# burlachenkok/flpytorch

Hardware: AMD Instinct MI355X
Metric: gradient-codec encode+reduce GB/s (device-resident), [N,D] fp32; % HBM peak (higher is better)
Workload: dtype f32; 1 GPU; C3 topk:1% N=1024/GPU D=10000000; codec=topk:1%, clients_per_gpu=1024, clients_total=1024, D=10000000, K=100000, rows_alloc=contiguous, parallelism=client-shard dp1

## Files before the change

### flpytorch_amd/csrc/select.hip

```cpp
#include <stdlib.h>

#include <atomic>
#include <map>
#include <mutex>
#include <vector>

#include "chunks.hpp"
#include "randk_tree.hpp"

namespace flc {

constexpr uint32_t ALL = 0xFFFFFFFFu;
constexpr uint32_t F_OVERFLOW = 1u, F_SHORT = 2u, F_TIES = 4u, F_EXACT = 8u;
constexpr uint32_t F_RESIDENT = 16u;
constexpr uint32_t F_REPAIR = 32u;
constexpr int SMAX = 16384;
constexpr int HBINS = 2048;
constexpr uint32_t TIECAP = HBINS;
constexpr int CS_SH = 64;
constexpr int64_t CS_FEW = 16;
constexpr int CS_ST = 8;
constexpr int CS_LCAP = 2048;
constexpr int RS_U = 16;
#ifndef FLC_RS_NG
// ... 3 lines not shown
constexpr int RS_NG_MAX = 16;
static_assert(RS_NG >= 1 && RS_NG <= RS_NG_MAX, "FLC_RS_NG: 1..16 groups");
constexpr int RS_GLOB = 0, RS_GEN = 32, RS_GAVE = 64, RS_CCNT = 96, RS_CDONE = 112, RS_GRP = 128;
constexpr int RS_XGRP = RS_GRP + 32 * RS_NG_MAX;
constexpr int RS_ABV = RS_XGRP + 32 * RS_NG_MAX;
constexpr int RS_CAP = 2048;
constexpr int RS_SS = 8192;
#ifndef FLC_RS_SR
#define FLC_RS_SR 1
#endif
constexpr int RS_SR = FLC_RS_SR;
#ifndef FLC_RS_STPOL
#define FLC_RS_STPOL 2
#endif
#ifndef FLC_RS_GACQ
#define FLC_RS_GACQ 1
#endif
#ifndef FLC_RS_POLLAB
#define FLC_RS_POLLAB 1
#endif
#ifndef FLC_RS_DONE
#define FLC_RS_DONE 1
#endif
#ifndef FLC_RS_RANKFIRST
#define FLC_RS_RANKFIRST 0
#endif
#ifndef FLC_RS_PROBE_NOCOUNT
#define FLC_RS_PROBE_NOCOUNT 0
#endif
#ifndef FLC_RS_G0REL
#define FLC_RS_G0REL 1
#endif
#ifndef FLC_RS_FENCE
#define FLC_RS_FENCE 0
#endif
#ifndef FLC_RS_SPEC
#define FLC_RS_SPEC 1
#endif
constexpr int RS_HREP = RS_ABV + 32 * RS_NG_MAX;
constexpr int RS_HSPEC = RS_HREP + 3 * RS_NG * HBINS;
constexpr int RS_CLIST = RS_HSPEC + 3 * RS_NG * HBINS;
constexpr int RS_TCNT = RS_CLIST + 2 * RS_CAP;
constexpr int RS_GMAX = 1024;
constexpr int RS_CS = 4;
constexpr int RS_CNUM = RS_TCNT + 2 * RS_GMAX;
constexpr int RS_CREG = RS_CNUM + RS_GMAX;
#ifdef FLC_RS_PRINT
constexpr int RS_PROBE = RS_CREG + 2 * RS_CS * RS_GMAX;
constexpr int RS_CTL = RS_PROBE + 4096;
#else
constexpr int RS_CTL = RS_CREG + 2 * RS_CS * RS_GMAX;
#endif
#ifndef FLC_RS_SPECST
#define FLC_RS_SPECST 0
#endif
#ifndef FLC_CS_LIST
#define FLC_CS_LIST 1
#endif
#ifndef FLC_CS_TWO_MAXD
#define FLC_CS_TWO_MAXD (int64_t(64) << 20)
#endif

struct SelWs {
    uint2* tab;
    uint32_t* ent_idx;
    float* ent_val;
    uint32_t* rowcnt;
    uint32_t* flags;
    uint32_t* thr;
    uint32_t* prefix;
    uint32_t* krem;
    uint32_t* tieprefix;
    uint32_t* tiecut;
    uint32_t* hist;
    uint32_t* worklist;
    uint32_t* nwork;
    uint32_t* cursor;
    uint32_t* cstate;
    uint64_t* clist;
    uint32_t* carrive;
    uint32_t* shcnt;
    uint32_t* zm;
    float* part;
    int64_t cap;
    uint32_t tie_hi;
};

__device__ __host__ inline uint32_t tie_pref(uint32_t ix, uint32_t hi) { return hi ? ix : ~ix; }
__device__ __host__ inline uint32_t tie_all(uint32_t hi) { return hi ? 0u : 0xFFFFFFFFu; }


__device__ inline void lds_bar() {
    asm volatile("s_waitcnt lgkmcnt(0)" ::: "memory");
    __builtin_amdgcn_s_barrier();
    asm volatile("" ::: "memory");
}
template <bool RAW>
__device__ inline void blk_bar() {
    if (RAW) lds_bar();
    else __syncthreads();
}
template <bool RAW = false>
__device__ inline void hist_find_at(const uint32_t* h, uint32_t k, uint32_t& bin, uint32_t& above,
                                    uint32_t* scratch , int t, bool own) {
    uint32_t local[8];
    uint32_t s = 0;
#pragma unroll
    for (int q = 0; q < 8; ++q) { local[q] = own ? h[HBINS - 1 - (t * 8 + q)] : 0u; s += local[q]; }
    if (t == 0) { scratch[256] = 0; scratch[257] = 0; }
    const int lane = t & 63, w = t >> 6;
    uint32_t inc = s;
#pragma unroll
    for (int off = 1; off < 64; off <<= 1) {
        const uint32_t v = __shfl_up(inc, off, 64);
        inc += lane >= off ? v : 0u;
    }
    if (own && lane == 63) scratch[w] = inc;
    blk_bar<RAW>();
    uint32_t before = 0;
    if (own)
        for (int q = 0; q < w; ++q) before += scratch[q];
    uint32_t incl = own ? before + inc : 0u, excl = incl - s;
    if (own && excl < k && incl >= k) {
        uint32_t run = excl;
#pragma unroll
        for (int q = 0; q < 8; ++q) {
            if (run + local[q] >= k) {
                scratch[256] = (uint32_t)(HBINS - 1 - (t * 8 + q));
                scratch[257] = run;
                break;
            }
            run += local[q];
        }
    }
    blk_bar<RAW>();
    bin = scratch[256];
    above = scratch[257];
    blk_bar<RAW>();
}
template <int NB>
__device__ inline void hist_find_n(const uint32_t* h, uint32_t k, uint32_t& bin, uint32_t& above, bool& found,
                                   uint32_t* scratch ) {
    constexpr int PER = NB / 256;
    static_assert(NB % 256 == 0, "256 threads scan NB / 256 bins each");
    const int t = (int)threadIdx.x;
    const bool own = t < 256;
    uint32_t local[PER];
    uint32_t s = 0;
#pragma unroll
    for (int q = 0; q < PER; ++q) { local[q] = own ? h[NB - 1 - (t * PER + q)] : 0u; s += local[q]; }
    if (t == 0) { scratch[256] = 0; scratch[257] = 0; scratch[258] = 0; }
    const int lane = t & 63, w = t >> 6;
    uint32_t inc = s;
#pragma unroll
    for (int off = 1; off < 64; off <<= 1) {
        const uint32_t v = __shfl_up(inc, off, 64);
        inc += lane >= off ? v : 0u;
    }
    if (own && lane == 63) scratch[w] = inc;
    __syncthreads();
    uint32_t before = 0;
    if (own)
        for (int q = 0; q < w; ++q) before += scratch[q];
    const uint32_t incl = own ? before + inc : 0u, excl = incl - s;
    if (own && excl < k && incl >= k) {
        uint32_t run = excl;
// ... 715 lines not shown
            __amdgpu_buffer_rsrc_t rsn;
            if (sub + 1 < FGS) {
                rsn = chunk_rsrc(rows.row_s(row), j0 + CHUNK, d);
            } else if (nit < items) {
                item_at(nit, nrow, nc);
                rsn = chunk_rsrc(rows.row_s(nrow), nc * CHUNK, d);
            } else {
                rsn = __builtin_amdgcn_make_buffer_rsrc(const_cast<float*>(rows.row_s(row)), (short)0, 0, 0x00020000);
            }
            const uint32_t cnt0 = cnt;
            __amdgpu_buffer_rsrc_t ro;
            if constexpr (LONE != 0) ro = chunk_rsrc(zout, j0, d);
            uint32_t lb = (uint32_t)j0 + (uint32_t)lane * 4u;
            asm volatile("" : "+v"(lb));
#pragma unroll
            for (int L = 0; L < 16; ++L) {
                const int P = L + RING - 1;
                ring[P % RING] = P < 16 ? load_q(rs, lane, P) : load_q(rsn, lane, P - 16);
                const float4 x = ring[L % RING];
                if constexpr (LONE != 0) {
                    typedef unsigned int u4v __attribute__((ext_vector_type(4)));
                    const u4v z = {0u, 0u, 0u, 0u};
                    __builtin_amdgcn_raw_buffer_store_b128(z, ro, lane * 16, L * 1024, 0);
                }
                const uint32_t jl = lb + (uint32_t)(L * 256);
                const float vq[4] = {x.x, x.y, x.z, x.w};
#pragma unroll
                for (int q = 0; q < 4; ++q) {
                    if (FLC_TK_PROBE == 3) { cnt += __float_as_uint(vq[q]) == 0x7F800001u ? 1u : 0u; continue; }
                    const bool f = mag_key(vq[q]) >= T;
                    const uint64_t m = __ballot(f);
                    if (FLC_TK_PROBE != 1 && f) {
                        const uint32_t pre = __builtin_amdgcn_mbcnt_hi((uint32_t)(m >> 32), __builtin_amdgcn_mbcnt_lo((uint32_t)m, 0u));
                        uint32_t sb = sla + min(cnt, (uint32_t)GCAP) * 4u;
                        asm volatile("" : "+s"(sb));
                        asm volatile("ds_write2st64_b32 %0, %1, %2 offset1:%3" ::"v"(sb + pre * 4u),
                                     "v"(jl + q), "v"(__float_as_uint(vq[q])), "i"(SROW * 4 / 256) : "memory");
                    }
                    cnt += (uint32_t)__popcll(m);
                }
            }
            ccp |= (uint64_t)min(cnt - cnt0, 0xFFFFu) << (16 * (c - cg0));
            rs = rsn;
        }
        if (pv) finish(par ^ 1);
        uint32_t res = 0;
        const int64_t shard = shards > 1 ? (cg0 / FGS) % shards : 0;
        if (cnt && cnt <= GCAP && lane == 0)
            res = atomicAdd(shards > 1 ? &ws.shcnt[(row * shards + shard) * RCS] : &ws.rowcnt[(row) * RCS], cnt);
        pv = true; prow = row; pc0 = cg0; pcc = ccp; ptot = cnt; pres = res; pseg = shard;
        __builtin_amdgcn_fence(__ATOMIC_SEQ_CST, "wavefront");
        par ^= 1;
        it = nit;
        row = nrow;
        c = nc;
    }
    __builtin_amdgcn_fence(__ATOMIC_SEQ_CST, "wavefront");
    finish(par ^ 1);
}

#ifndef FLC_TK_WG
#define FLC_TK_WG 1
#endif
#ifndef FLC_TK_WG_NL
#define FLC_TK_WG_NL 4
#endif
#ifndef FLC_TK_WG_RING
#define FLC_TK_WG_RING FLC_TK_RING
#endif
#ifndef FLC_TK_WG_STPOL
#define FLC_TK_WG_STPOL 17
#endif
#ifndef FLC_TK_WG_WPE
#define FLC_TK_WG_WPE 4
#endif
__device__ inline uint32_t lds_addr(const void* p) {
    return (uint32_t)(size_t)(const __attribute__((address_space(3))) void*)p;
}
__device__ inline uint32_t lds_peek(uint32_t addr) {
    uint32_t v;
    asm volatile("ds_read_b32 %0, %1\n\ts_waitcnt lgkmcnt(0)" : "=&v"(v) : "v"(addr) : "memory");
    return __builtin_amdgcn_readfirstlane(v);
}
template <int RING, int NL>
__global__ __launch_bounds__((NL + 1) * 64) __attribute__((amdgpu_waves_per_eu(FLC_TK_WG_WPE))) void k_topk_filter_fast_wg(RowSrc rows, int64_t n, int64_t r0, int64_t rn, int64_t rb, int64_t d,
                                                                        SelWs ws) {
    static_assert(16 % RING == 0, "ring must divide the 16 loads of a chunk");
    constexpr int FGS = 4;
    constexpr int SROW = GCAP + 64;
    __shared__ __attribute__((aligned(16))) uint32_t st[2][NL][2 * SROW];
    __shared__ __attribute__((aligned(16))) uint32_t hs[2][NL][4];
    __shared__ uint32_t fr[2];
    const int lane = threadIdx.x & 63;
    const int wv = __builtin_amdgcn_readfirstlane(threadIdx.x >> 6);
    if (threadIdx.x < 2 * NL * 4) (&hs[0][0][0])[threadIdx.x] = 0;
    if (threadIdx.x < 2) fr[threadIdx.x] = 0;
    __syncthreads();
    const int64_t C = nchunks(d);
    const int64_t G = (C + FGS * NL - 1) / (FGS * NL);
    const int64_t items = rn * G;
    const int64_t stride = gridDim.x;
    int64_t it = blockIdx.x;
    if (it >= items) return;
    auto item_at = [&](int64_t t, int64_t& r, int64_t& cc) {
        const int64_t blk = t / (rb * G), rem = t - blk * rb * G;
        const int64_t bn = min(rb, rn - blk * rb);
        const int64_t g = rem / bn;
        r = r0 + blk * rb + (rem - g * bn);
        cc = g * (FGS * NL);
    };
    if (wv == NL) {
        for (uint32_t k = 0; it < items; it += stride, ++k) {
            const int b = k & 1;
            int64_t row, c0;
            item_at(it, row, c0);
            const uint32_t fa = lds_addr(&hs[b][min(lane, NL - 1)][3]);
            for (;;) {
                uint32_t f;
                asm volatile("ds_read_b32 %0, %1\n\ts_waitcnt lgkmcnt(0)" : "=&v"(f) : "v"(fa) : "memory");
                if (__ballot(f != k + 1) == 0) break;
                __builtin_amdgcn_s_sleep(4);
            }
            uint32_t pre[NL], tot[NL], sum = 0;
            uint64_t cc[NL];
            bool allfit = true;
#pragma unroll
            for (int w = 0; w < NL; ++w) {
                const uint4 h = *reinterpret_cast<const uint4*>(hs[b][w]);
                cc[w] = (uint64_t)h.x | ((uint64_t)h.y << 32);
                tot[w] = h.z;
                pre[w] = sum;
                sum += tot[w] <= GCAP ? tot[w] : 0u;
                allfit = allfit && tot[w] <= GCAP;
            }
            uint32_t base = 0;
            bool fits = true;
            if (sum) {
                uint32_t res = 0;
                if (lane == 0) res = atomicAdd(&ws.rowcnt[row * RCS], sum);
                base = __shfl(res, 0, WAVE);
                fits = (int64_t)base + sum <= ws.cap;
            }
            if (lane < FGS * NL && c0 + lane < C) {
                uint32_t off = 0, cu = 0;
                bool gf = false;
#pragma unroll
                for (int w = 0; w < NL; ++w)
                    if ((lane >> 2) == w) {
                        off = pre[w];
                        gf = tot[w] <= GCAP;
#pragma unroll
                        for (int u = 0; u < FGS; ++u) {
                            const uint32_t x = (uint32_t)(cc[w] >> (16 * u)) & 0xFFFFu;
                            off += u < (lane & 3) ? x : 0u;
                            cu = u == (lane & 3) ? x : cu;
                        }
                    }
                ws.tab[(c0 + lane) * n + row] = make_uint2(base + off, fits && gf ? cu : 0u);
            }
            if (!(fits && allfit) && lane == 0) atomicOr(&ws.flags[row], F_OVERFLOW);
#pragma unroll
            for (int w = 0; w < NL; ++w)
                tk_copy_out<FLC_TK_WG_STPOL>(st[b][w], st[b][w] + SROW, ws, n, row, base + pre[w], tot[w], fits && tot[w] <= GCAP, lane,
                            (int64_t)blockIdx.x * NL + w);
            asm volatile("s_waitcnt lgkmcnt(0)\n\tds_write_b32 %0, %1" ::"v"(lds_addr(&fr[b])), "v"(k + 1) : "memory");
        }
        return;
    }
    float4 ring[RING];
    int64_t row, c;
    item_at(it, row, c);
    c += wv * FGS;
    auto rs = chunk_rsrc(rows.row_s(row), c * CHUNK, d);
#pragma unroll
    for (int L = 0; L < RING - 1; ++L) {
        ring[L] = load_q(rs, lane, L);
        __builtin_amdgcn_sched_barrier(0);
    }
    for (uint32_t k = 0; it < items; ++k) {
        const int b = k & 1;
        if (k >= 2) {
            const uint32_t fa = lds_addr(&fr[b]);
            while (lds_peek(fa) != k - 1) __builtin_amdgcn_s_sleep(2);
        }
        const uint32_t T = max(sload(ws.thr + row), 1u);
        const int64_t nit = it + stride;
        const uint32_t sla = __builtin_amdgcn_readfirstlane(lds_addr(st[b][wv]));
        uint32_t cnt = 0;
        uint64_t ccp = 0;
        const int64_t cg0 = c;
        int64_t nrow = row, nc = c;
#pragma unroll
        for (int sub = 0; sub < FGS; ++sub, ++c) {
            const int64_t j0 = c * CHUNK;
            __amdgpu_buffer_rsrc_t rsn;
            if (sub + 1 < FGS) {
                rsn = chunk_rsrc(rows.row_s(row), j0 + CHUNK, d);
            } else if (nit < items) {
                item_at(nit, nrow, nc);
                nc += wv * FGS;
                rsn = chunk_rsrc(rows.row_s(nrow), nc * CHUNK, d);
            } else {
                rsn = __builtin_amdgcn_make_buffer_rsrc(const_cast<float*>(rows.row_s(row)), (short)0, 0, 0x00020000);
            }
            const uint32_t cnt0 = cnt;
            uint32_t lb = (uint32_t)j0 + (uint32_t)lane * 4u;
            asm volatile("" : "+v"(lb));
#pragma unroll
            for (int L = 0; L < 16; ++L) {
                const int P = L + RING - 1;
                ring[P % RING] = P < 16 ? load_q(rs, lane, P) : load_q(rsn, lane, P - 16);
                const float4 x = ring[L % RING];
                const uint32_t jl = lb + (uint32_t)(L * 256);
                const float vq[4] = {x.x, x.y, x.z, x.w};
#pragma unroll
                for (int q = 0; q < 4; ++q) {
                    const bool f = mag_key(vq[q]) >= T;
                    const uint64_t m = __ballot(f);
                    if (f) {
                        const uint32_t pre = __builtin_amdgcn_mbcnt_hi((uint32_t)(m >> 32), __builtin_amdgcn_mbcnt_lo((uint32_t)m, 0u));
                        uint32_t sb = sla + min(cnt, (uint32_t)GCAP) * 4u;
                        asm volatile("" : "+s"(sb));
                        asm volatile("ds_write2st64_b32 %0, %1, %2 offset1:%3" ::"v"(sb + pre * 4u),
                                     "v"(jl + q), "v"(__float_as_uint(vq[q])), "i"(SROW * 4 / 256) : "memory");
                    }
                    cnt += (uint32_t)__popcll(m);
                }
            }
            ccp |= (uint64_t)min(cnt - cnt0, 0xFFFFu) << (16 * (c - cg0));
            rs = rsn;
        }
        if (lane == 0)
            asm volatile("ds_write_b64 %0, %1\n\tds_write_b32 %0, %2 offset:8\n\tds_write_b32 %0, %3 offset:12"
                         ::"v"(lds_addr(hs[b][wv])), "v"(ccp), "v"(cnt), "v"(k + 1) : "memory");
        it = nit;
        row = nrow;
        c = nc;
    }
}

template <bool FULLROW>
__global__ __launch_bounds__(256) void k_radix_hist(RowSrc rows, int64_t n, int64_t d, int p, SelWs ws) {
    __shared__ uint32_t h[HBINS];
    constexpr int64_t BLK = 65536;
    const int64_t nrows = FULLROW ? (int64_t)(*ws.nwork) : n;
    const int64_t maxlen = FULLROW ? d : ws.cap;
    const int64_t bpr = (maxlen + BLK - 1) / BLK;
    const int64_t items = nrows * bpr;
// ... 1884 lines not shown
            }
            const u4v ov = {o[0], o[1], o[2], o[3]};
            __builtin_amdgcn_raw_buffer_store_b128(ov, ro, voff, u * RS_NT * 16, FLC_RS_STPOL);
        }
    }
    RS_STAMP(11);
    (void)bar;
    }
    goto done;
leave:
    if (t == 0) {
        __builtin_amdgcn_fence(__ATOMIC_RELEASE, "agent");
    }
    if (!rep_s) count_out();
    __syncthreads();
    if (rep_s) {
        const RsExit ex = ex_s;
        if (t == 0) {
            const uint64_t t0 = (uint64_t)wall_clock64();
            for (;;) {
                uint32_t out_n = 0;
                for (int r = 0; r < RS_NG; ++r)
                    out_n += __hip_atomic_load(ex.ctl + RS_XGRP + 32 * r, __ATOMIC_RELAXED, __HIP_MEMORY_SCOPE_AGENT);
                if (out_n - ex.xbase >= ex.G - 1u || (uint64_t)wall_clock64() - t0 >= 64 * ex.spin) break;
                __builtin_amdgcn_s_sleep(8);
            }
            __builtin_amdgcn_fence(__ATOMIC_ACQUIRE, "agent");
        }
        __syncthreads();
        rs_repair(ex.x, ex.d, ex.K, ex.tie_hi, ex.thr, ex.krem, ex.tiecut, ex.flags, ex.out, ex.ctl, h, scratch, wsum);
        __syncthreads();
        if (t == 0) __builtin_amdgcn_fence(__ATOMIC_RELEASE, "agent");
        count_out();
    }
done:;
#ifdef FLC_RS_PRINT
    asm volatile("s_waitcnt vmcnt(0)" ::: "memory");
    __syncthreads();
    RS_STAMP(12);
    if (t == 0 && G <= 256u) {
        uint64_t* pr = reinterpret_cast<uint64_t*>(ex_s.ctl + RS_PROBE);
        const int ks[8] = {FLC_RS_TLK, 13};
        for (int k = 0; k < 8; ++k) __hip_atomic_store(pr + k * 256 + g, stamp[ks[k]], __ATOMIC_RELAXED, __HIP_MEMORY_SCOPE_AGENT);
    }
#endif
}

static int64_t host_chunks(int64_t d) { return (d + CHUNK - 1) / CHUNK; }

int64_t sel_capacity(int codec, int64_t d, int64_t K) {
    if (codec == FLC_RANDK) return std::max<int64_t>(K, 1);
    int64_t cap = 2 * K + 2 * CHUNK;
    cap = std::min<int64_t>(std::max<int64_t>(cap, 1), std::max<int64_t>(d, 1));
    return (cap + 3) & ~int64_t(3);
}

static SelWs carve_sel(void* base, int codec, int64_t n, int64_t d, int64_t K, size_t* bytes) {
    Carver cv(base);
    const int64_t C = std::max<int64_t>(host_chunks(d), 1), nn = std::max<int64_t>(n, 1);
    SelWs s;
    s.tie_hi = 0;
    s.cap = sel_capacity(codec, d, K);
    s.tab = cv.take<uint2>((size_t)C * nn);
    s.ent_idx = cv.take<uint32_t>((size_t)nn * s.cap);
    s.ent_val = cv.take<float>((size_t)nn * s.cap);
    s.rowcnt = cv.take<uint32_t>((size_t)nn * RCS);
    s.flags = cv.take<uint32_t>(nn);
    s.thr = cv.take<uint32_t>(nn);
    s.prefix = cv.take<uint32_t>(nn);
    s.krem = cv.take<uint32_t>(nn);
    s.worklist = cv.take<uint32_t>(nn);
    s.nwork = cv.take<uint32_t>(4);
    s.zm = cv.take<uint32_t>((size_t)C * (CHUNK / 32));
    s.part = codec == FLC_TOPK ? cv.take<float>((size_t)C * CHUNK) : nullptr;
    if (codec == FLC_TOPK) {
        s.tieprefix = cv.take<uint32_t>((size_t)C * nn);
        s.tiecut = cv.take<uint32_t>(nn);
        s.hist = cv.take<uint32_t>((size_t)nn * HBINS);
        s.cursor = nullptr;
        s.cstate = cv.take<uint32_t>((size_t)nn * CS_ST);
        s.clist = cv.take<uint64_t>((size_t)std::min<int64_t>(nn, CS_FEW) * CS_LCAP);
        s.carrive = cv.take<uint32_t>((size_t)nn * RCS);
        s.shcnt = cv.take<uint32_t>((size_t)std::min<int64_t>(nn, CS_FEW) * CS_SH * RCS);
    } else {
        s.tieprefix = nullptr;
        s.tiecut = nullptr;
        s.hist = nullptr;
        s.cursor = cv.take<uint32_t>((size_t)std::max<int64_t>(C, RK_SB) * nn);
        s.cstate = nullptr;
        s.clist = nullptr;
        s.carrive = nullptr;
        s.shcnt = nullptr;
    }
    if (bytes) *bytes = cv.bytes();
    return s;
}

size_t randk_device_workspace(int64_t n, int64_t d);

size_t sel_workspace(const flc_codec_params* prm, int64_t n, int64_t d) {
    size_t b = 0;
    carve_sel(nullptr, prm->codec, n, d, prm->k, &b);
    if (prm->codec == FLC_RANDK) b += randk_device_workspace(n, d);
    return b;
}

static int grid_stride_blocks(int64_t items, int64_t cap = 4096) {
    return (int)std::max<int64_t>(1, std::min<int64_t>(items, cap));
}

static int accum_parts() {
    static const int p = [] {
        const char* e = tuning_env("FLC_ACCUM_PARTS");
        const int v = e ? atoi(e) : 0;
        return (v == 1 || v == 2 || v == 4) ? v : 0;
    }();
    return p;
}

static bool assign_fold() {
    static const bool v = [] { const char* e = tuning_env("FLC_ASSIGN_FOLD"); return e && atoi(e) == 1; }();
    return v;
}

static bool cs_single() {
    static const bool v = [] { const char* e = tuning_env("FLC_CS_SINGLE"); return e && atoi(e) == 1; }();
    return v;
}

#ifndef FLC_LONE_PATH
#define FLC_LONE_PATH 2
#endif
#ifndef FLC_RS_EVREC
#define FLC_RS_EVREC 1
#endif
#ifndef FLC_RS_COOP
#define FLC_RS_COOP 0
#endif
struct RsCtx {
    uint32_t* ctl = nullptr;
    uint32_t seq = 0;
    uint32_t xcum = 0;
    hipStream_t last = nullptr;
    hipEvent_t done = nullptr;
};
static std::mutex g_rs_mu;
static std::map<int, RsCtx> g_rs_ctx;
static std::atomic<int> g_rs_dbg_mult{1};
static std::atomic<long long> g_rs_dbg_spin{0};
int rs_debug(int mult, int64_t spin_ticks) {
    if (mult < 1 || mult > 64 || spin_ticks < 0) { set_error("flc_debug_resident: mult 1..64, spin >= 0"); return FLC_ERR_ARG; }
    g_rs_dbg_mult.store(mult);
    g_rs_dbg_spin.store((long long)spin_ticks);
    return FLC_OK;
}
static int rs_cus() {
    static int cu[64] = {0};
    int dev = 0;
    if (hipGetDevice(&dev) != hipSuccess || dev < 0 || dev >= 64) return 0;
    if (!cu[dev]) {
        int c = 0;
        if (hipDeviceGetAttribute(&c, hipDeviceAttributeMultiprocessorCount, dev) != hipSuccess) return 0;
        cu[dev] = c;
    }
    return cu[dev];
}
static int lone_path() {
    static const int v = [] { const char* e = tuning_env("FLC_LONE_PATH"); return e ? atoi(e) : FLC_LONE_PATH; }();
    return v;
}

static int filter_group() {
    static const int g = [] {
        const char* e = tuning_env("FLC_FILTER_GS");
        return (e && atoi(e) == 2) ? 2 : 4;
    }();
    return g;
}

template <int FGS>
static void launch_filter(RowSrc rows, int64_t n, int64_t r0, int64_t rn, int64_t d, SelWs ws, hipStream_t st,
                          int shards, float* zout = nullptr) {
    const int64_t waves = rn * ((nchunks(d) + FGS - 1) / FGS);
    const int gw = (int)std::max<int64_t>(1, std::min<int64_t>((waves + 3) / 4, 32768));
    static const int64_t rb = [] {
        const char* e = tuning_env("FLC_TK_RB");
        return e ? std::max<int64_t>(1, atoll(e)) : (int64_t)64;
    }();
    ProfScope _pv(FGS == 4 ? "k_topk_filter_g4" : "k_topk_filter_g2", st);
    if constexpr (FGS == 4 && FLC_TK_WG != 0 && FLC_TK_PROBE != 1 && FLC_TK_PROBE != 3) {
        static const bool wg = [] { const char* e = tuning_env("FLC_FILTER_WG"); return !(e && atoi(e) == 0); }();
        if (wg && shards == 1 && !zout) {
            constexpr int NL = FLC_TK_WG_NL;
            const int64_t items = rn * ((nchunks(d) + 4 * NL - 1) / (4 * NL));
            const int gi = (int)std::max<int64_t>(1, std::min<int64_t>(items, 32768));
            static const int64_t rbw = [] {
                const char* e = tuning_env("FLC_TK_RB");
                return e ? std::max<int64_t>(1, atoll(e)) : (int64_t)16;
            }();
            hipLaunchKernelGGL((k_topk_filter_fast_wg<FLC_TK_WG_RING, NL>), dim3(gi), dim3((NL + 1) * 64), 0, st, rows, n, r0,
                               rn, std::min(rbw, std::max<int64_t>(rn, 1)), d, ws);
            return;
        }
    }
    if (zout)
        hipLaunchKernelGGL((k_topk_filter_fast<FLC_TK_RING, FGS, 1>), dim3(gw), dim3(256), 0, st, rows, n, r0, rn,
                           std::min(rb, std::max<int64_t>(rn, 1)), d, ws, shards, zout);
    else
        hipLaunchKernelGGL((k_topk_filter_fast<FLC_TK_RING, FGS>), dim3(gw), dim3(256), 0, st, rows, n, r0, rn,
                           std::min(rb, std::max<int64_t>(rn, 1)), d, ws, shards, (float*)nullptr);
}

#ifndef FLC_TK_SPLIT_SAMPLE
#define FLC_TK_SPLIT_SAMPLE 1
#endif
#ifndef FLC_TK_LASTPCT
#define FLC_TK_LASTPCT 100
#endif
static_assert(FLC_TK_LASTPCT >= 1 && FLC_TK_LASTPCT <= 100, "FLC_TK_LASTPCT: the last row group is 1..100 % of the others");
#ifndef FLC_TK_LAST_TS
#define FLC_TK_LAST_TS 4096
#endif
#ifndef FLC_TK_GFOLD
#define FLC_TK_GFOLD 1
#endif
#ifndef FLC_TK_SIDE_NT
#define FLC_TK_SIDE_NT 512
#endif
#ifndef FLC_TK_EXACT_WG
#define FLC_TK_EXACT_WG 256
#endif
static int tk_tail_groups(const flc_codec_params* prm, int64_t n) {
    static const int g = [] { const char* e = tuning_env("FLC_TK_TAILOV"); return e ? std::max(1, atoi(e)) : 4; }();
    const int hint = (prm->flags >> 8) & 0xFF;
    if (hint) return (int)std::max<int64_t>(1, std::min<int64_t>(hint, n));
    return (int)std::max<int64_t>(1, std::min<int64_t>(g, n / 64));
}
namespace {
struct TkCtx {
    hipStream_t side = nullptr;
    std::vector<hipEvent_t> ev;
};
std::mutex g_tk_mu;
std::map<int, TkCtx> g_tk_ctx;
}

static int launch_chunk_accum(int64_t n, int64_t d, SelWs ws, bool assign, const float* w, float wt, float* out,
                              hipStream_t st);

static RkdWs carve_rkd(void* base, int64_t n, int64_t d, size_t* bytes) {
    Carver cv(base);
    const int64_t C = std::max<int64_t>(host_chunks(d), 1), nn = std::max<int64_t>(n, 1);
    RkdWs s;
    s.cnt = cv.take<uint32_t>((size_t)C * nn);
    s.ckey = cv.take<uint64_t>((size_t)nn);
    if (bytes) *bytes = cv.bytes();
    return s;
}

size_t randk_device_workspace(int64_t n, int64_t d) {
    size_t b = 0;
    carve_rkd(nullptr, n, d, &b);
    return b;
}

static int randk_counts(const flc_codec_params* prm, const flc_pattern* pat, int64_t n, int64_t d, RkdWs ws,
                        hipStream_t st) {
    ProfScope _ps("k_randk_counts", st);
    const int64_t parts = (host_chunks(d) + RKC_BINS - 1) / RKC_BINS;
    hipLaunchKernelGGL(k_randk_counts, dim3((unsigned)parts, (unsigned)n), dim3(RKC_NT), 0, st, n, d, prm->k, prm->seed,
                       pat ? pat->client0 : (int64_t)0, ws);
    FLC_CHECK_LAUNCH("k_randk_counts");
    return FLC_OK;
}

static int randk_counts_or_given(const flc_codec_params* prm, const flc_pattern* pat, int64_t n, int64_t d, RkdWs* rw,
                                 hipStream_t st) {
    if (pat && pat->d_randk_counts) {
        rw->cnt = const_cast<uint32_t*>(pat->d_randk_counts);
        hipLaunchKernelGGL(k_randk_ckeys, dim3((unsigned)((n + 255) / 256)), dim3(256), 0, st, n, prm->seed,
                           pat->client0, rw->ckey);
        FLC_CHECK_LAUNCH("k_randk_ckeys");
        return FLC_OK;
    }
    return randk_counts(prm, pat, n, d, *rw, st);
}

int randk_device_prepare(const flc_codec_params* prm, const flc_pattern* pat, int64_t n, int64_t d, void* wsp,
                         const uint32_t** cnt, const uint64_t** ckey, hipStream_t st) {
    RkdWs rw = carve_rkd(wsp, n, d, nullptr);
    if (int rc = randk_counts_or_given(prm, pat, n, d, &rw, st)) return rc;
    *cnt = rw.cnt;
    *ckey = rw.ckey;
    return FLC_OK;
}

int randk_device_counts(uint64_t seed, int64_t client0, int64_t n, int64_t d, int64_t k, uint32_t* cnt, void* wsp,
                        size_t ws_bytes, hipStream_t st) {
    if (ws_bytes < randk_device_workspace(n, d)) { set_error("randk counts: workspace too small"); return FLC_ERR_WORKSPACE; }
    RkdWs ws = carve_rkd(wsp, n, d, nullptr);
    ws.cnt = cnt;
    flc_codec_params prm{};
    prm.codec = FLC_RANDK;
    prm.k = k;
    prm.seed = seed;
    flc_pattern pat{};
    pat.client0 = client0;
    return randk_counts(&prm, &pat, n, d, ws, st);
}

int randk_device_run(const flc_codec_params* prm, const flc_pattern* pat, RowSrc rows, int64_t n, int64_t d,
                     const float* w, float wt, float* out, void* wsp, size_t ws_bytes, hipStream_t st) {
    size_t lb = 0;
    carve_sel(nullptr, FLC_RANDK, n, d, prm->k, &lb);
    if (ws_bytes < lb + randk_device_workspace(n, d)) { set_error("randk: workspace too small"); return FLC_ERR_WORKSPACE; }
    SelWs sw = carve_sel(wsp, FLC_RANDK, n, d, prm->k, nullptr);
    RkdWs rw = carve_rkd(static_cast<char*>(wsp) + lb, n, d, nullptr);
    const int64_t C = host_chunks(d);
    auto counts = [&]() -> int { return randk_counts_or_given(prm, pat, n, d, &rw, st); };
    if (C >= 1024) {
        if (int rc = counts()) return rc;
        ProfScope _ps("k_randk_fold", st);
        const int ab = grid_stride_blocks((C + 3) / 4, 16384);
        hipLaunchKernelGGL((k_randk_fold<CHUNK>), dim3(ab), dim3(256), 0, st, rows, n, d, rw.cnt, rw.ckey,
                           prm->randk_scale, w, wt, out);
        FLC_CHECK_LAUNCH("k_randk_fold");
        return FLC_OK;
// ... 101 lines not shown

static int sel_run_impl(const flc_codec_params* prm, const flc_pattern* pat, RowSrc rows, bool vec, int64_t n, int64_t d,
                        bool assign, const float* w, float wt, float* out, void* wsp, size_t ws_bytes, hipStream_t st,
                        bool lists_only) {
    const int codec = prm->codec;
    const int64_t K = prm->k;
    if (d == 0) return FLC_OK;
    if (n == 0) { FLC_CHECK_HIP(hipMemsetAsync(out, 0, (size_t)d * sizeof(float), st)); return FLC_OK; }
    if (K < 1 || K > d) { set_error("K=%lld outside [1, D=%lld]", (long long)K, (long long)d); return FLC_ERR_ARG; }
    if (d >= (int64_t)0xFFFFFFFF) { set_error("D too large for 32-bit entry indices"); return FLC_ERR_ARG; }
    if (codec == FLC_RANDK && !(pat && pat->d_randk_idx))
        return randk_device_run(prm, pat, rows, n, d, w, wt, out, wsp, ws_bytes, st);
    size_t need = 0;
    carve_sel(nullptr, codec, n, d, K, &need);
    if (ws_bytes < need) { set_error("select: workspace %zu < %zu", ws_bytes, need); return FLC_ERR_WORKSPACE; }
    SelWs ws = carve_sel(wsp, codec, n, d, K, nullptr);
    if (codec == FLC_TOPK) {
        if (prm->tie != FLC_TIE_LOWEST && prm->tie != FLC_TIE_HIGHEST) { set_error("topk: unknown tie rule %d", prm->tie); return FLC_ERR_ARG; }
        ws.tie_hi = prm->tie == FLC_TIE_HIGHEST ? 1u : 0u;
    }
    const int64_t C = host_chunks(d);
    bool lone_assign = false, gfold = false;
    const bool few = codec == FLC_TOPK && n <= CS_FEW && !cs_single() && sel_capacity(codec, d, K) >= (int64_t)CS_SH * GCAP;
    if (codec == FLC_RANDK) {
        if (int rc = randk_lists_launch(prm, pat, rows, n, d, ws, st)) return rc;
    } else {
        hipStreamCaptureStatus cap = hipStreamCaptureStatusNone;
        if (assign && n == 1 && !assign_fold() && lone_path() == 2) FLC_CHECK_HIP(hipStreamIsCapturing(st, &cap));
        if (assign && n == 1 && !assign_fold() && lone_path() == 2 && cap == hipStreamCaptureStatusNone) {
            const int64_t cus = rs_cus();
            const int mult = std::max(1, g_rs_dbg_mult.load());
            const int64_t G = std::min<int64_t>(cus * mult, (d + RS_NT * 4 - 1) / (RS_NT * 4));
            const int64_t e4 = G > 0 ? (d + G * RS_NT * 4 - 1) / (G * RS_NT * 4) : RS_U + 1;
            if (e4 <= RS_U && d * 4 < ((int64_t)1 << 31)) {
                const int64_t Gu = (d + e4 * RS_NT * 4 - 1) / (e4 * RS_NT * 4);
                const long long dspin = g_rs_dbg_spin.load();
                const uint64_t spin = dspin > 0 ? (uint64_t)dspin : (uint64_t)FLC_RS_SPIN;
                ProfScope _ps("k_lone_resident", st);
                int dev = 0;
                FLC_CHECK_HIP(hipGetDevice(&dev));
                std::lock_guard<std::mutex> lk(g_rs_mu);
                RsCtx& rc = g_rs_ctx[dev];
                if (!rc.ctl) {
                    FLC_CHECK_HIP(hipMalloc(reinterpret_cast<void**>(&rc.ctl), (size_t)RS_CTL * sizeof(uint32_t)));
                    FLC_CHECK_HIP(hipMemsetAsync(rc.ctl, 0, (size_t)RS_CTL * sizeof(uint32_t), st));
                    FLC_CHECK_HIP(hipEventCreateWithFlags(&rc.done, FLC_SYNC_EVENT_FLAGS));
                }
                if (rc.last && rc.last != st) {
                    if (!FLC_RS_EVREC) FLC_CHECK_HIP(hipEventRecord(rc.done, rc.last));
                    FLC_CHECK_HIP(hipStreamWaitEvent(st, rc.done, 0));
                }
                if (++rc.seq == 0u) rc.seq = 1u;
                const int e4i = (int)e4;
                if (FLC_RS_COOP) {
                    RowSrc ra = rows;
                    int64_t da = d, ka = K;
                    SelWs wa = ws;
                    float* oa = out;
                    int ea = e4i;
                    uint32_t* ca = rc.ctl;
                    uint32_t sa = rc.seq;
                    uint64_t pa = spin;
                    uint32_t xa = rc.xcum;
                    void* args[] = {&ra, &da, &ka, &wa, &oa, &ea, &ca, &sa, &pa, &xa};
                    FLC_CHECK_HIP(hipLaunchCooperativeKernel(reinterpret_cast<const void*>(&k_lone_resident<RS_U>), dim3((unsigned)Gu),
                                                             dim3(RS_NT), args, 0, st));
                } else {
                    hipLaunchKernelGGL((k_lone_resident<RS_U>), dim3((unsigned)Gu), dim3(RS_NT), 0, st, rows, d, K, ws, out, e4i,
                                       rc.ctl, rc.seq, spin, rc.xcum);
                }
                FLC_CHECK_LAUNCH("k_lone_resident");
                rc.xcum += (uint32_t)Gu;
                if (FLC_RS_EVREC) FLC_CHECK_HIP(hipEventRecord(rc.done, st));
                rc.last = st;
                return FLC_OK;
            }
        }
        const bool dense_k = K * 16 > d;
        lone_assign = assign && n == 1 && few && !dense_k && !assign_fold();

        if (dense_k) FLC_CHECK_HIP(hipMemsetAsync(ws.hist, 0, (size_t)n * HBINS * sizeof(uint32_t), st));
        const int64_t bpr = (C + 3) / 4;
        if (!dense_k) {
            const int TG = few ? 1 : tk_tail_groups(prm, n);
            gfold = FLC_TK_GFOLD && !few && !assign && !dense_k && !lists_only;
            hipStream_t sside = st;
            TkCtx* cx = nullptr;
            std::unique_lock<std::mutex> lk;
            if (TG > 1) {
                int dev = 0;
                FLC_CHECK_HIP(hipGetDevice(&dev));
                lk = std::unique_lock<std::mutex>(g_tk_mu);
                cx = &g_tk_ctx[dev];
                if (!cx->side) {
                    int lo = 0, hi = 0;
                    FLC_CHECK_HIP(hipDeviceGetStreamPriorityRange(&lo, &hi));
                    FLC_CHECK_HIP(hipStreamCreateWithPriority(&cx->side, hipStreamNonBlocking, hi));
                }
                while ((int)cx->ev.size() < TG + 3) {
                    hipEvent_t e;
                    FLC_CHECK_HIP(hipEventCreateWithFlags(&e, FLC_SYNC_EVENT_FLAGS));
                    cx->ev.push_back(e);
                }
                sside = cx->side;
            }
            const bool split = FLC_TK_SPLIT_SAMPLE && TG > 1;
            const int64_t rs1 = split ? group_row(n, TG, 1, FLC_TK_LASTPCT) : n;
            auto sample = [&](int64_t a, int64_t b, hipStream_t sx) {
                if (b <= a) return;
                ProfScope _ps("k_topk_sample", sx);
                hipLaunchKernelGGL((few ? k_topk_sample<1024, true> : k_topk_sample<1024, false>), dim3((unsigned)(b - a)), dim3(1024), 0, sx,
                                   rows, n, d, K, ws, few ? 1 : 0, a);
            };
            if (split) {
                FLC_CHECK_HIP(hipEventRecord(cx->ev[TG + 1], st));
                FLC_CHECK_HIP(hipStreamWaitEvent(sside, cx->ev[TG + 1], 0));
            }
            sample(0, rs1, st);
            FLC_CHECK_LAUNCH("k_topk_sample");
            if (split) {
                sample(rs1, n, sside);
                FLC_CHECK_LAUNCH("k_topk_sample (side)");
                FLC_CHECK_HIP(hipEventRecord(cx->ev[TG + 2], sside));
            }
            for (int g = 0; g < TG; ++g) {
                const int64_t r0 = group_row(n, TG, g, FLC_TK_LASTPCT), rn = group_row(n, TG, g + 1, FLC_TK_LASTPCT) - r0;
                if (split && g == 1) FLC_CHECK_HIP(hipStreamWaitEvent(st, cx->ev[TG + 2], 0));
                { ProfScope _ps("k_topk_filter", st);
                float* zout = lone_assign ? out : nullptr;
                if (filter_group() == 2 || n * d < ((int64_t)64 << 20)) launch_filter<2>(rows, n, r0, rn, d, ws, st, few ? CS_SH : 1, zout);
                else launch_filter<4>(rows, n, r0, rn, d, ws, st, few ? CS_SH : 1, zout); }
                FLC_CHECK_LAUNCH("k_topk_filter");
                if (TG > 1) {
                    FLC_CHECK_HIP(hipEventRecord(cx->ev[g], st));
                    FLC_CHECK_HIP(hipStreamWaitEvent(sside, cx->ev[g], 0));
                }
                { ProfScope _ps("k_cand_select", sside);
                if (few) {
                    const int np = (FLC_CS_LIST && d <= FLC_CS_TWO_MAXD) ? 2 : 3;
                    for (int p = 0; p < np; ++p)
                        hipLaunchKernelGGL(k_cs_pass, dim3((unsigned)CS_SH, (unsigned)n), dim3(CS_NT), 0, st, K, ws,
                                           p == np - 1 ? 1 : 0);
                } else if (gfold) {
                    const bool big = rn < 128 || g == TG - 1;
                    const int nt = big ? 1024 : FLC_TK_SIDE_NT;
                    const dim3 grid((unsigned)(big ? rn : grid_stride_blocks(rn, 8192)));
                    if (big) {
                        if (vec) hipLaunchKernelGGL((k_cand_select_x<1024, true>), grid, dim3(nt), 0, sside, rows, n, r0, rn, d, K, ws);
                        else hipLaunchKernelGGL((k_cand_select_x<1024, false>), grid, dim3(nt), 0, sside, rows, n, r0, rn, d, K, ws);
                    } else if (FLC_TK_SIDE_NT == 256) {
                        if (vec) hipLaunchKernelGGL((k_cand_select_x<256, true>), grid, dim3(nt), 0, sside, rows, n, r0, rn, d, K, ws);
                        else hipLaunchKernelGGL((k_cand_select_x<256, false>), grid, dim3(nt), 0, sside, rows, n, r0, rn, d, K, ws);
                    } else {
                        if (vec) hipLaunchKernelGGL((k_cand_select_x<512, true>), grid, dim3(nt), 0, sside, rows, n, r0, rn, d, K, ws);
                        else hipLaunchKernelGGL((k_cand_select_x<512, false>), grid, dim3(nt), 0, sside, rows, n, r0, rn, d, K, ws);
                    }
                } else if (rn < 128 || (TG > 1 && g == TG - 1))
                    hipLaunchKernelGGL(k_cand_select<1024>, dim3((unsigned)rn), dim3(1024), 0, sside, r0, rn, K, ws);
                else if (FLC_TK_SIDE_NT == 256)
                    hipLaunchKernelGGL(k_cand_select<256>, dim3(grid_stride_blocks(rn, 8192)), dim3(256), 0, sside, r0, rn, K, ws);
                else hipLaunchKernelGGL(k_cand_select<512>, dim3(grid_stride_blocks(rn, 8192)), dim3(512), 0, sside, r0, rn, K, ws); }
                FLC_CHECK_LAUNCH("k_cand_select");
                if (gfold) {
                    const bool lastg = g == TG - 1;
                    if (int rc = launch_group_fold(n, d, ws, w, wt, out, r0, r0 + rn, g == 0, lastg, lastg || TG == 1, sside))
                        return rc;
                }
            }
            if (!lone_assign && !gfold) {
                ProfScope _ps("k_topk_exact_rows", sside);
                const int eb = grid_stride_blocks(n, FLC_TK_EXACT_WG);
                if (vec) hipLaunchKernelGGL((k_topk_exact_rows<true>), dim3(eb), dim3(EX_NT), 0, sside, rows, n, (int64_t)0, n, d, K, ws);
                else hipLaunchKernelGGL((k_topk_exact_rows<false>), dim3(eb), dim3(EX_NT), 0, sside, rows, n, (int64_t)0, n, d, K, ws);
                FLC_CHECK_LAUNCH("k_topk_exact_rows");
            }
            if (TG > 1) {
                FLC_CHECK_HIP(hipEventRecord(cx->ev[TG], sside));
                FLC_CHECK_HIP(hipStreamWaitEvent(st, cx->ev[TG], 0));
            }
        } else {
            FLC_CHECK_HIP(hipMemsetAsync(ws.flags, 0, (size_t)n * sizeof(uint32_t), st));
        }
        if (dense_k) {
        hipLaunchKernelGGL(k_build_worklist, dim3(1), dim3(1024), 0, st, n, K, d, ws, 1);
        FLC_CHECK_LAUNCH("k_build_worklist");
        const int64_t hb = (d + 65535) / 65536;
        for (int p = 0; p < 3; ++p) {
            { ProfScope _ps("k_radix_hist_full", st);
hipLaunchKernelGGL((k_radix_hist<true>), dim3(grid_stride_blocks(n * hb)), dim3(256), 0, st, rows, n, d, p, ws); }
            FLC_CHECK_LAUNCH("k_radix_hist(full)");
            hipLaunchKernelGGL((k_radix_select<true>), dim3(grid_stride_blocks(n, 1024)), dim3(256), 0, st, n, p, K, ws);
            FLC_CHECK_LAUNCH("k_radix_select(full)");
        }
        hipLaunchKernelGGL(k_tie_count, dim3(grid_stride_blocks(n * bpr, 4096)), dim3(256), 0, st, rows, n, d, ws);
        FLC_CHECK_LAUNCH("k_tie_count");
        hipLaunchKernelGGL(k_tie_scan, dim3(grid_stride_blocks(n, 1024)), dim3(256), 0, st, n, d, ws);
        FLC_CHECK_LAUNCH("k_tie_scan");
        int gb = grid_stride_blocks(n * bpr, 8192);
        { ProfScope _ps("k_topk_filter_exact", st);
if (vec) hipLaunchKernelGGL((k_topk_filter<true, true>), dim3(gb), dim3(256), 0, st, rows, n, d, ws);
        else hipLaunchKernelGGL((k_topk_filter<true, false>), dim3(gb), dim3(256), 0, st, rows, n, d, ws); }
        FLC_CHECK_LAUNCH("k_topk_filter(exact)");
        }
    }
    if (lists_only) return FLC_OK;
    if (lone_assign) {
        ProfScope _ps("k_assign_finish", st);
        if (vec) hipLaunchKernelGGL((k_assign_finish<true>), dim3(CS_SH), dim3(EX_NT), 0, st, rows, d, K, ws, out);
        else hipLaunchKernelGGL((k_assign_finish<false>), dim3(CS_SH), dim3(EX_NT), 0, st, rows, d, K, ws, out);
        FLC_CHECK_LAUNCH("k_assign_finish");
        return FLC_OK;
    }
    if (gfold) return FLC_OK;
    if (assign && n == 1 && codec == FLC_TOPK && !assign_fold()) {
        FLC_CHECK_HIP(hipMemsetAsync(out, 0, (size_t)d * sizeof(float), st));
        const int sb = (int)std::max<int64_t>(1, std::min<int64_t>((sel_capacity(codec, d, K) + 255) / 256, 2048));
        hipLaunchKernelGGL(k_assign_scatter, dim3(sb), dim3(256), 0, st, ws, out, few ? 1 : 0);
        FLC_CHECK_LAUNCH("k_assign_scatter");
        return FLC_OK;
    }
    return launch_chunk_accum(n, d, ws, assign, w, wt, out, st);
}

int sel_run(const flc_codec_params* prm, const flc_pattern* pat, RowSrc rows, bool vec, int64_t n, int64_t d,
            bool assign, const float* w, float wt, float* out, void* wsp, size_t ws_bytes, hipStream_t st) {
    return sel_run_impl(prm, pat, rows, vec, n, d, assign, w, wt, out, wsp, ws_bytes, st, false);
}

int topk_lists_build(const flc_codec_params* prm, RowSrc rows, bool vec, int64_t n, int64_t d, void* wsp, size_t ws_bytes,
                     TkLists* lists, hipStream_t st) {
    if (prm->codec != FLC_TOPK) { set_error("topk_lists_build: TopK only"); return FLC_ERR_ARG; }
    if (int rc = sel_run_impl(prm, nullptr, rows, vec, n, d, false, nullptr, 1.f, nullptr, wsp, ws_bytes, st, true))
        return rc;
    const SelWs ws = carve_sel(wsp, FLC_TOPK, n, d, prm->k, nullptr);
    lists->tab = ws.tab;
    lists->ent_idx = ws.ent_idx;
    lists->ent_val = ws.ent_val;
    lists->cap = ws.cap;
    lists->thr = ws.thr;
    lists->flags = ws.flags;
    lists->tiecut = ws.tiecut;
    lists->tie_hi = prm->tie == FLC_TIE_HIGHEST ? 1u : 0u;
    return FLC_OK;
}

int topk_lists_fold(const flc_codec_params* prm, int64_t n, int64_t d, void* wsp, const float* w, float wt, float* out,
                    hipStream_t st) {
    SelWs ws = carve_sel(wsp, FLC_TOPK, n, d, prm->k, nullptr);
    ws.tie_hi = prm->tie == FLC_TIE_HIGHEST ? 1u : 0u;
    return launch_chunk_accum(n, d, ws, false, w, wt, out, st);
}

int sel_row_flags(const flc_codec_params* prm, int64_t n, int64_t d, const void* wsp, size_t ws_bytes,
                  uint32_t* flags, hipStream_t st) {
    if (prm->codec != FLC_TOPK) { set_error("flc_select_row_flags: TopK only"); return FLC_ERR_ARG; }
    if (n <= 0 || d <= 0) return FLC_OK;
    size_t need = 0;
    carve_sel(nullptr, prm->codec, n, d, prm->k, &need);
    if (ws_bytes < need) { set_error("flc_select_row_flags: workspace %zu < %zu", ws_bytes, need); return FLC_ERR_WORKSPACE; }
    const SelWs ws = carve_sel(const_cast<void*>(wsp), prm->codec, n, d, prm->k, nullptr);
    FLC_CHECK_HIP(hipMemcpyAsync(flags, ws.flags, (size_t)n * sizeof(uint32_t), hipMemcpyDeviceToDevice, st));
    return FLC_OK;
// ... 96 lines not shown
```

Before: 5905 GB/s.

## Fuse per-group top-k filter launches into one kernel with device-side group signals

```diff
diff --git a/flpytorch_amd/csrc/select.hip b/flpytorch_amd/csrc/select.hip
--- a/flpytorch_amd/csrc/select.hip
+++ b/flpytorch_amd/csrc/select.hip
@@ -109,6 +109,7 @@
     uint32_t* shcnt;
     uint32_t* zm;
     float* part;
+    uint32_t* gdone;
     int64_t cap;
     uint32_t tie_hi;
 };
@@ -990,9 +991,25 @@
     asm volatile("ds_read_b32 %0, %1\n\ts_waitcnt lgkmcnt(0)" : "=&v"(v) : "v"(addr) : "memory");
     return __builtin_amdgcn_readfirstlane(v);
 }
-template <int RING, int NL>
+constexpr int TK_GMAX = 8;
+struct TkGroups {
+    int ng;
+    uint32_t seq;
+    int64_t row[TK_GMAX + 1];
+    uint64_t* sig[TK_GMAX];
+    uint32_t* gdone;
+};
+__host__ __device__ inline int64_t tk_group_items(int64_t rn, int64_t d, int NL) {
+    return rn * ((nchunks(d) + 4 * NL - 1) / (4 * NL));
+}
+#ifndef FLC_TK_ONE_BLOCKS
+#define FLC_TK_ONE_BLOCKS 32768
+#endif
+__host__ __device__ inline int64_t tk_group_blocks(int64_t items) { return items < FLC_TK_ONE_BLOCKS ? items : FLC_TK_ONE_BLOCKS; }
+
+template <int RING, int NL, bool ONE = false>
 __global__ __launch_bounds__((NL + 1) * 64) __attribute__((amdgpu_waves_per_eu(FLC_TK_WG_WPE))) void k_topk_filter_fast_wg(RowSrc rows, int64_t n, int64_t r0, int64_t rn, int64_t rb, int64_t d,
-                                                                        SelWs ws) {
+                                                                        SelWs ws, TkGroups tg) {
     static_assert(16 % RING == 0, "ring must divide the 16 loads of a chunk");
     constexpr int FGS = 4;
     constexpr int SROW = GCAP + 64;
@@ -1006,9 +1023,34 @@
     __syncthreads();
     const int64_t C = nchunks(d);
     const int64_t G = (C + FGS * NL - 1) / (FGS * NL);
-    const int64_t items = rn * G;
-    const int64_t stride = gridDim.x;
     int64_t it = blockIdx.x;
+    int64_t stride = gridDim.x;
+    uint32_t* gdone = nullptr;
+    uint64_t* gsig = nullptr;
+    if constexpr (ONE) {
+        bool found = false;
+        const int64_t rbw = rb;
+#pragma unroll
+        for (int g = 0; g < TK_GMAX; ++g) {
+            const int64_t gn = tg.row[g + 1] - tg.row[g];
+            const int64_t nb = tk_group_blocks(tk_group_items(gn, d, NL));
+            if (g < tg.ng && !found) {
+                if (it < nb) {
+                    found = true;
+                    r0 = tg.row[g];
+                    rn = gn;
+                    rb = min(rbw, gn);
+                    stride = nb;
+                    gdone = tg.gdone + g;
+                    gsig = tg.sig[g];
+                } else {
+                    it -= nb;
+                }
+            }
+        }
+        if (!found) return;
+    }
+    const int64_t items = ONE ? tk_group_items(rn, d, NL) : rn * G;
     if (it >= items) return;
     auto item_at = [&](int64_t t, int64_t& r, int64_t& cc) {
         const int64_t blk = t / (rb * G), rem = t - blk * rb * G;
@@ -1064,7 +1106,11 @@
                             cu = u == (lane & 3) ? x : cu;
                         }
                     }
-                ws.tab[(c0 + lane) * n + row] = make_uint2(base + off, fits && gf ? cu : 0u);
+                const uint2 te = make_uint2(base + off, fits && gf ? cu : 0u);
+                if constexpr (ONE)
+                    __hip_atomic_store(reinterpret_cast<uint64_t*>(&ws.tab[(c0 + lane) * n + row]), (uint64_t)te.x | ((uint64_t)te.y << 32),
+                                       __ATOMIC_RELAXED, __HIP_MEMORY_SCOPE_AGENT);
+                else ws.tab[(c0 + lane) * n + row] = te;
             }
             if (!(fits && allfit) && lane == 0) atomicOr(&ws.flags[row], F_OVERFLOW);
 #pragma unroll
@@ -1072,6 +1118,15 @@
                 tk_copy_out<FLC_TK_WG_STPOL>(st[b][w], st[b][w] + SROW, ws, n, row, base + pre[w], tot[w], fits && tot[w] <= GCAP, lane,
                             (int64_t)blockIdx.x * NL + w);
             asm volatile("s_waitcnt lgkmcnt(0)\n\tds_write_b32 %0, %1" ::"v"(lds_addr(&fr[b])), "v"(k + 1) : "memory");
+            if constexpr (ONE) {
+                asm volatile("s_waitcnt vmcnt(0)" ::: "memory");
+                if (lane == 0 &&
+                    __hip_atomic_fetch_add(gdone, 1u, __ATOMIC_RELAXED, __HIP_MEMORY_SCOPE_AGENT) + 1u == (uint32_t)items) {
+                    __builtin_amdgcn_fence(__ATOMIC_ACQ_REL, "");
+                    asm volatile("s_waitcnt vmcnt(0)" ::: "memory");
+                    __hip_atomic_store(gsig, (uint64_t)tg.seq, __ATOMIC_RELAXED, __HIP_MEMORY_SCOPE_SYSTEM);
+                }
+            }
         }
         return;
     }
@@ -3122,7 +3177,9 @@
         s.clist = cv.take<uint64_t>((size_t)std::min<int64_t>(nn, CS_FEW) * CS_LCAP);
         s.carrive = cv.take<uint32_t>((size_t)nn * RCS);
         s.shcnt = cv.take<uint32_t>((size_t)std::min<int64_t>(nn, CS_FEW) * CS_SH * RCS);
+        s.gdone = cv.take<uint32_t>(TK_GMAX);
     } else {
+        s.gdone = nullptr;
         s.tieprefix = nullptr;
         s.tiecut = nullptr;
         s.hist = nullptr;
@@ -3218,6 +3275,14 @@
     return g;
 }
 
+static int64_t tk_wg_rb() {
+    static const int64_t rbw = [] {
+        const char* e = tuning_env("FLC_TK_RB");
+        return e ? std::max<int64_t>(1, atoll(e)) : (int64_t)16;
+    }();
+    return rbw;
+}
+
 template <int FGS>
 static void launch_filter(RowSrc rows, int64_t n, int64_t r0, int64_t rn, int64_t d, SelWs ws, hipStream_t st,
                           int shards, float* zout = nullptr) {
@@ -3234,12 +3299,9 @@
             constexpr int NL = FLC_TK_WG_NL;
             const int64_t items = rn * ((nchunks(d) + 4 * NL - 1) / (4 * NL));
             const int gi = (int)std::max<int64_t>(1, std::min<int64_t>(items, 32768));
-            static const int64_t rbw = [] {
-                const char* e = tuning_env("FLC_TK_RB");
-                return e ? std::max<int64_t>(1, atoll(e)) : (int64_t)16;
-            }();
+            const int64_t rbw = tk_wg_rb();
             hipLaunchKernelGGL((k_topk_filter_fast_wg<FLC_TK_WG_RING, NL>), dim3(gi), dim3((NL + 1) * 64), 0, st, rows, n, r0,
-                               rn, std::min(rbw, std::max<int64_t>(rn, 1)), d, ws);
+                               rn, std::min(rbw, std::max<int64_t>(rn, 1)), d, ws, TkGroups{});
             return;
         }
     }
@@ -3280,9 +3342,77 @@
 struct TkCtx {
     hipStream_t side = nullptr;
     std::vector<hipEvent_t> ev;
+    int can_wait = -1;
+    uint64_t* sig[TK_GMAX] = {};
+    uint32_t seq = 0;
+    hipStream_t last = nullptr;
+    hipEvent_t done = nullptr;
 };
 std::mutex g_tk_mu;
 std::map<int, TkCtx> g_tk_ctx;
+}
+
+#ifndef FLC_TK_ONELAUNCH
+#define FLC_TK_ONELAUNCH 1
+#endif
+#ifndef FLC_TK_FLOOR
+#define FLC_TK_FLOOR 64
+#endif
+#ifndef FLC_TK_FLOOR_DIV
+#define FLC_TK_FLOOR_DIV 16
+#endif
+#ifndef FLC_TK_ONE_SMALL512
+#define FLC_TK_ONE_SMALL512 1
+#endif
+static int tk_onelaunch() {
+    static const int v = [] { const char* e = tuning_env("FLC_TK_ONELAUNCH"); return e ? atoi(e) : FLC_TK_ONELAUNCH; }();
+    return v;
+}
+static int64_t tk_floor() {
+    static const int64_t v = [] { const char* e = tuning_env("FLC_TK_FLOOR"); return e ? (int64_t)atoll(e) : (int64_t)FLC_TK_FLOOR; }();
+    return v;
+}
+static int tk_group_table(int64_t n, int TG, bool taper, int64_t* b) {
+    int G = 0;
+    b[0] = 0;
+    const int64_t floor = tk_floor() < 1 ? 0 : std::max<int64_t>(tk_floor(), n / FLC_TK_FLOOR_DIV);
+    if (!taper || floor < 1 || TG < 2) {
+        for (int g = 1; g <= TG; ++g) b[g] = group_row(n, TG, g, FLC_TK_LASTPCT);
+        return TG;
+    }
+    for (int g = 1; g < TG; ++g) b[++G] = group_row(n, TG, g, 100);
+    int64_t r = n - b[G];
+    while (r >= 2 * floor && G + 2 <= TK_GMAX) {
+        const int64_t h = (r + 1) / 2;
+        b[G + 1] = b[G] + h;
+        ++G;
+        r -= h;
+    }
+    b[++G] = n;
+    return G;
+}
+
+static void launch_filter_groups(RowSrc rows, int64_t n, int64_t d, SelWs ws, hipStream_t st, const int64_t* b, int g0, int g1,
+                                 uint64_t* const* sig, uint32_t seq) {
+    constexpr int NL = FLC_TK_WG_NL;
+    TkGroups tg{};
+    tg.ng = g1 - g0;
+    tg.seq = seq;
+    tg.gdone = ws.gdone + g0;
+    int64_t blocks = 0;
+    for (int g = g0; g <= g1; ++g) tg.row[g - g0] = b[g];
+    for (int g = g1 - g0 + 1; g <= TK_GMAX; ++g) tg.row[g] = b[g1];
+    for (int g = g0; g < g1; ++g) {
+        tg.sig[g - g0] = sig[g];
+        blocks += tk_group_blocks(tk_group_items(b[g + 1] - b[g], d, NL));
+    }
+    if (blocks == 0) return;
+    int scopes = 0;
+    for (int g = g0; g < g1; ++g) scopes += b[g + 1] > b[g] ? 1 : 0;
+    for (int s = 1; s < scopes; ++s) { ProfScope _pe("k_topk_filter_g4", st); }
+    ProfScope _pv("k_topk_filter_g4", st);
+    hipLaunchKernelGGL((k_topk_filter_fast_wg<FLC_TK_WG_RING, NL, true>), dim3((unsigned)blocks), dim3((NL + 1) * 64), 0, st, rows, n,
+                       (int64_t)0, (int64_t)0, tk_wg_rb(), d, ws, tg);
 }
 
 static int launch_chunk_accum(int64_t n, int64_t d, SelWs ws, bool assign, const float* w, float wt, float* out,
@@ -3550,12 +3680,13 @@
         if (dense_k) FLC_CHECK_HIP(hipMemsetAsync(ws.hist, 0, (size_t)n * HBINS * sizeof(uint32_t), st));
         const int64_t bpr = (C + 3) / 4;
         if (!dense_k) {
-            const int TG = few ? 1 : tk_tail_groups(prm, n);
+            const int TG0 = few ? 1 : tk_tail_groups(prm, n);
             gfold = FLC_TK_GFOLD && !few && !assign && !dense_k && !lists_only;
             hipStream_t sside = st;
             TkCtx* cx = nullptr;
             std::unique_lock<std::mutex> lk;
-            if (TG > 1) {
+            bool one = false;
+            if (TG0 > 1) {
                 int dev = 0;
                 FLC_CHECK_HIP(hipGetDevice(&dev));
                 lk = std::unique_lock<std::mutex>(g_tk_mu);
@@ -3565,15 +3696,50 @@
                     FLC_CHECK_HIP(hipDeviceGetStreamPriorityRange(&lo, &hi));
                     FLC_CHECK_HIP(hipStreamCreateWithPriority(&cx->side, hipStreamNonBlocking, hi));
                 }
-                while ((int)cx->ev.size() < TG + 3) {
+                while ((int)cx->ev.size() < std::max(TG0, TK_GMAX) + 3) {
                     hipEvent_t e;
                     FLC_CHECK_HIP(hipEventCreateWithFlags(&e, FLC_SYNC_EVENT_FLAGS));
                     cx->ev.push_back(e);
                 }
                 sside = cx->side;
-            }
-            const bool split = FLC_TK_SPLIT_SAMPLE && TG > 1;
-            const int64_t rs1 = split ? group_row(n, TG, 1, FLC_TK_LASTPCT) : n;
+                static const bool wgk = [] { const char* e = tuning_env("FLC_FILTER_WG"); return !(e && atoi(e) == 0); }();
+                one = FLC_TK_WG != 0 && FLC_TK_PROBE != 1 && FLC_TK_PROBE != 3 && wgk && tk_onelaunch() != 0 && TG0 <= TK_GMAX &&
+                      filter_group() != 2 && n * d >= ((int64_t)64 << 20) &&
+                      tk_group_items(n, d, FLC_TK_WG_NL) < ((int64_t)1 << 32);
+                if (one) {
+                    hipStreamCaptureStatus cs = hipStreamCaptureStatusNone;
+                    FLC_CHECK_HIP(hipStreamIsCapturing(st, &cs));
+                    one = cs == hipStreamCaptureStatusNone;
+                }
+                if (one && cx->can_wait < 0) {
+                    int v = 0;
+                    if (hipDeviceGetAttribute(&v, hipDeviceAttributeCanUseStreamWaitValue, dev) != hipSuccess) v = 0;
+                    for (int g = 0; g < TK_GMAX && v; ++g) {
+                        void* p = nullptr;
+                        if (hipExtMallocWithFlags(&p, sizeof(uint64_t), hipMallocSignalMemory) != hipSuccess) { v = 0; break; }
+                        cx->sig[g] = static_cast<uint64_t*>(p);
+                        if (hipStreamWriteValue64(st, p, 0, 0) != hipSuccess) v = 0;
+                    }
+                    if (v && hipEventCreateWithFlags(&cx->done, FLC_SYNC_EVENT_FLAGS) != hipSuccess) v = 0;
+                    if (!v) (void)hipGetLastError();
+                    cx->can_wait = v;
+                }
+                one = one && cx->can_wait == 1;
+                if (one && cx->last && cx->last != st) FLC_CHECK_HIP(hipStreamWaitEvent(st, cx->done, 0));
+                if (one) {
+                    if (cx->seq == 0xFFFFFFFFu) {
+                        FLC_CHECK_HIP(hipDeviceSynchronize());
+                        for (int g = 0; g < TK_GMAX; ++g) FLC_CHECK_HIP(hipStreamWriteValue64(st, cx->sig[g], 0, 0));
+                        cx->seq = 0;
+                    }
+                    ++cx->seq;
+                    FLC_CHECK_HIP(hipMemsetAsync(ws.gdone, 0, TK_GMAX * sizeof(uint32_t), st));
+                }
+            }
+            int64_t gb[256 + 2];
+            const int TG = tk_group_table(n, TG0, one && ((prm->flags >> 8) & 0xFF) == 0, gb);
+            const bool split = FLC_TK_SPLIT_SAMPLE && TG > 1 && !(one && tk_onelaunch() == 2);
+            const int64_t rs1 = split ? gb[1] : n;
             auto sample = [&](int64_t a, int64_t b, hipStream_t sx) {
                 if (b <= a) return;
                 ProfScope _ps("k_topk_sample", sx);
@@ -3591,8 +3757,26 @@
                 FLC_CHECK_LAUNCH("k_topk_sample (side)");
                 FLC_CHECK_HIP(hipEventRecord(cx->ev[TG + 2], sside));
             }
+            if (one) {
+                const int g1 = split ? 1 : 0;
+                if (g1) {
+                    ProfScope _ps("k_topk_filter", st);
+                    launch_filter_groups(rows, n, d, ws, st, gb, 0, g1, cx->sig, cx->seq);
+                    FLC_CHECK_LAUNCH("k_topk_filter");
+                    FLC_CHECK_HIP(hipStreamWaitEvent(st, cx->ev[TG + 2], 0));
+                }
+                { ProfScope _ps("k_topk_filter", st);
+                ProfScope _po("k_topk_filter_one", st);
+                launch_filter_groups(rows, n, d, ws, st, gb, g1, TG, cx->sig, cx->seq); }
+                FLC_CHECK_LAUNCH("k_topk_filter");
+                for (int g = 0; g < TG; ++g)
+                    if (gb[g + 1] > gb[g]) FLC_CHECK_HIP(hipStreamWriteValue32(st, cx->sig[g], cx->seq, 0));
+            }
             for (int g = 0; g < TG; ++g) {
-                const int64_t r0 = group_row(n, TG, g, FLC_TK_LASTPCT), rn = group_row(n, TG, g + 1, FLC_TK_LASTPCT) - r0;
+                const int64_t r0 = gb[g], rn = gb[g + 1] - r0;
+                if (one) {
+                    if (rn > 0) FLC_CHECK_HIP(hipStreamWaitValue32(sside, cx->sig[g], cx->seq, hipStreamWaitValueGte, 0xFFFFFFFFu));
+                } else {
                 if (split && g == 1) FLC_CHECK_HIP(hipStreamWaitEvent(st, cx->ev[TG + 2], 0));
                 { ProfScope _ps("k_topk_filter", st);
                 float* zout = lone_assign ? out : nullptr;
@@ -3603,6 +3787,7 @@
                     FLC_CHECK_HIP(hipEventRecord(cx->ev[g], st));
                     FLC_CHECK_HIP(hipStreamWaitEvent(sside, cx->ev[g], 0));
                 }
+                }
                 { ProfScope _ps("k_cand_select", sside);
                 if (few) {
                     const int np = (FLC_CS_LIST && d <= FLC_CS_TWO_MAXD) ? 2 : 3;
@@ -3610,7 +3795,7 @@
                         hipLaunchKernelGGL(k_cs_pass, dim3((unsigned)CS_SH, (unsigned)n), dim3(CS_NT), 0, st, K, ws,
                                            p == np - 1 ? 1 : 0);
                 } else if (gfold) {
-                    const bool big = rn < 128 || g == TG - 1;
+                    const bool big = (rn < 128 && !(one && FLC_TK_ONE_SMALL512)) || g == TG - 1;
                     const int nt = big ? 1024 : FLC_TK_SIDE_NT;
                     const dim3 grid((unsigned)(big ? rn : grid_stride_blocks(rn, 8192)));
                     if (big) {
@@ -3646,6 +3831,10 @@
                 FLC_CHECK_HIP(hipEventRecord(cx->ev[TG], sside));
                 FLC_CHECK_HIP(hipStreamWaitEvent(st, cx->ev[TG], 0));
             }
+            if (one) {
+                FLC_CHECK_HIP(hipEventRecord(cx->done, st));
+                cx->last = st;
+            }
         } else {
             FLC_CHECK_HIP(hipMemsetAsync(ws.flags, 0, (size_t)n * sizeof(uint32_t), st));
         }
```

Result: no change. 5914 GB/s, median of 2 (+0.1%).
